# nv-tlabs/DefTet

Measured on AMD Instinct MI355X. Metric: M tet-point tests/s (fwd+bwd) at res=70, 100k queries, higher is better.
Workload: dtype f32

## Files before the change

deftet_amd/csrc/point_in_tet.hip:

```cpp
#pragma clang fp contract(off)

#include <stdlib.h>

#include <algorithm>
#include <type_traits>
#include <vector>

#include "common.hpp"
#include "wave.hpp"

namespace deftet {
namespace pit {

constexpr float kBig = 1048576.0f;
constexpr float kTau = 1.0f / 128.0f;
constexpr float kMargin = 1.0f / 64.0f;
constexpr float kWMin = 9.3132257e-10f;
constexpr int kMiss = 0x7F7F7F7F;
constexpr int kMaxG = 112;
constexpr int kMaxBins = 15 * 1024;
constexpr int kHitOverflow = -2;

constexpr int kHitPad = 64;
__host__ __device__ inline int hit_pad(int B) { return (B + kHitPad - 1) / kHitPad * kHitPad; }
__host__ __device__ inline size_t hit_cnt_off(int B, int T) { return (size_t)B * T * 2; }
__host__ __device__ inline size_t hit_list_off(int B, int T) { return (size_t)B * T * 2 + (size_t)3 * hit_pad(B); }
__host__ __device__ inline size_t hit_spill_off(int B, int T, int Q) { return (hit_list_off(B, T) + (size_t)B * Q + 3) / 4 * 4; }
constexpr int kHitSpilled = 1 << 30;
constexpr int kRecSlots = 2, kSpillSlots = 4;
constexpr int kOvfCap = 128;
__device__ __forceinline__ void note_overflow(int *counters, int nB, int b, int t)
{
    counters[b * 4 + 2] = 1;
    const int k = atomicAdd(&counters[nB * 4 + b * 4 + 2], 1);
    if (k < kOvfCap) counters[nB * 8 + b * kOvfCap + k] = t;
}

__device__ __forceinline__ void put_hit_record(int2 *hits, int4 *spill, size_t idx, const int (&hq)[kRecSlots + kSpillSlots], int n,
                                               int *counters, int nB, int b, int t)
{
    if (n > kRecSlots + kSpillSlots || (n > kRecSlots && !spill)) {
        hits[idx] = make_int2(-1, kHitOverflow);
        note_overflow(counters, nB, b, t);
        return;
    }
    if (n > kRecSlots) spill[idx] = make_int4(hq[2], hq[3], hq[4], hq[5]);
    hits[idx] = make_int2(n > kRecSlots ? (hq[0] | kHitSpilled) : hq[0], hq[1]);
}

#ifdef PIT_PHASE_TIMING
constexpr int kPhaseWaves = 1 << 17;
__device__ unsigned long long g_phase[kPhaseWaves][16];
#define PHASE_DECL                                                                                      \
    long long ph_t_ = clock64();                                                                        \
    const unsigned ph_w_ = (((unsigned)blockIdx.y * gridDim.x + blockIdx.x) * 4u + (threadIdx.x >> 6)) & (kPhaseWaves - 1)
#define PHASE_MARK(i)                                                                  \
    do {                                                                               \
        const long long ph_n_ = clock64();                                             \
        if ((threadIdx.x & 63) == 0) g_phase[ph_w_][i] += (unsigned long long)(ph_n_ - ph_t_); \
        ph_t_ = ph_n_;                                                                 \
    } while (0)
#define PHASE_COUNT(i, v)                                                              \
    do {                                                                               \
        const unsigned long long pc_ = (unsigned long long)(v);                        \
        if ((threadIdx.x & 63) == 0) g_phase[ph_w_][i] += pc_;                         \
    } while (0)
__device__ unsigned long long g_span[kPhaseWaves][2];
#define SPAN_MARK(k)                                                                                                     \
    do {                                                                                                                 \
        if ((threadIdx.x & 63) == 0) g_span[ph_w_][k] = wall_clock64();                                                  \
    } while (0)
__device__ unsigned long long g_reason[8];
#define REASON_COUNT(i, mask)                                                                                        \
    do {                                                                                                             \
        const unsigned long long rm_ = (mask);                                                                       \
        if (rm_ != 0ull && (threadIdx.x & 63) == 0) atomicAdd(&g_reason[i], (unsigned long long)__popcll(rm_));     \
    } while (0)
#else
#define SPAN_MARK(k)
#define REASON_COUNT(i, mask)
#define PHASE_DECL
#define PHASE_MARK(i)
#define PHASE_COUNT(i, v)
#endif

struct Planes {
    float n[4][3];
// ... 160 lines not shown

__device__ __forceinline__ bool query_regular(float x, float y, float z)
{
    return fabsf(x) <= kBig && fabsf(y) <= kBig && fabsf(z) <= kBig;
}

__host__ __device__ inline int table_pitch(int G) { return G + 3; }
__device__ __forceinline__ unsigned table_off(int cz, int cx, int cy, int Gx, int Gp)
{
    return (unsigned)((cz * (Gx + 1) + cx) * Gp + cy);
}

__global__ __launch_bounds__(256) void k_query_bbox(const float *__restrict__ pts, int Q, float *part, int *counters,
                                                    int *result, int nB, long long nQ)
{
    __shared__ float sh[4][6];
    const int b = blockIdx.y;
    {
        const long long nblk = (long long)gridDim.x * gridDim.y, bid = (long long)blockIdx.y * gridDim.x + blockIdx.x;
        const long long i = bid * blockDim.x + threadIdx.x, stride = nblk * blockDim.x;
        if (i < nB * 8) counters[i] = 0;
        for (long long j = i; j < nQ; j += stride) result[j] = kMiss;
    }
    const float *p = pts + (size_t)b * Q * 3;
    float lo[3] = {INFINITY, INFINITY, INFINITY}, hi[3] = {-INFINITY, -INFINITY, -INFINITY};
    constexpr int kBoxKeep = 8;
    const int stride = gridDim.x * blockDim.x;
    for (int q0 = blockIdx.x * blockDim.x + threadIdx.x; q0 < Q; q0 += stride * kBoxKeep) {
        float x[kBoxKeep], y[kBoxKeep], z[kBoxKeep];
#pragma unroll
        for (int k = 0; k < kBoxKeep; ++k) {
            const float *pq = p + (size_t)min(q0 + k * stride, Q - 1) * 3;
            x[k] = pq[0]; y[k] = pq[1]; z[k] = pq[2];
        }
#pragma unroll
        for (int k = 0; k < kBoxKeep; ++k)
            if (query_regular(x[k], y[k], z[k])) {
                lo[0] = fminf(lo[0], x[k]); lo[1] = fminf(lo[1], y[k]); lo[2] = fminf(lo[2], z[k]);
                hi[0] = fmaxf(hi[0], x[k]); hi[1] = fmaxf(hi[1], y[k]); hi[2] = fmaxf(hi[2], z[k]);
            }
    }
#pragma unroll
    for (int off = 32; off > 0; off >>= 1) {
#pragma unroll
        for (int k = 0; k < 3; ++k) {
            lo[k] = fminf(lo[k], __shfl_xor(lo[k], off));
            hi[k] = fmaxf(hi[k], __shfl_xor(hi[k], off));
        }
    }
    const int w = threadIdx.x >> 6;
    if ((threadIdx.x & 63) == 0) {
#pragma unroll
        for (int k = 0; k < 3; ++k) { sh[w][k] = lo[k]; sh[w][3 + k] = hi[k]; }
    }
    __syncthreads();
    if (threadIdx.x < 6) {
        const int k = threadIdx.x;
        float v = sh[0][k];
        for (int i = 1; i < 4; ++i) v = k < 3 ? fminf(v, sh[i][k]) : fmaxf(v, sh[i][k]);
        part[((size_t)b * kBoxBlocks + blockIdx.x) * 6 + k] = v;
    }
}

__device__ __forceinline__ int2 shape_block(int pin)
{
    if (!pin) return make_int2(blockIdx.y, blockIdx.x);
    const int L = blockIdx.y * gridDim.x + blockIdx.x, nB = gridDim.y;
    return make_int2(L % nB, L / nB);
}
static inline int pin_shapes(int Q) { return (size_t)Q * 36 <= ((size_t)4 << 20); }

constexpr int kMaxRowBlocks = 256;
#ifndef PIT_ROWTILE
#define PIT_ROWTILE 2048
#endif
constexpr int kRowTile = PIT_ROWTILE;
#ifndef PIT_LOCAL_THREADS
#define PIT_LOCAL_THREADS 512
#endif
constexpr int kLocalThreads = PIT_LOCAL_THREADS;
constexpr int kLocalWaves = kLocalThreads / 64;
constexpr int kLocalKeep = kRowTile / kLocalThreads;
static_assert(kLocalThreads % 64 == 0 && kLocalKeep * kLocalThreads == kRowTile, "whole waves, whole trips over a chunk");
constexpr int kSub = 4;
constexpr int kParts = 4;
constexpr int kSubPerPart = kSub / kParts;
constexpr int kMaxBin1 = kMaxG * kSub;

template <bool HINT>
__global__ __launch_bounds__(kLocalThreads) void k_slab_local(const float *__restrict__ pts, int Q, const float *__restrict__ bboxPart,
                                                    float *gparam, int G, int Gx, int nblk, int prePitch, int chunkQ,
                                                    float4 *localQ, int *pre, int *counters, int *irregQ,
                                                    const float *__restrict__ boxIn, float *partOut, int *irrCnt, int *result)
{
    __shared__ int hist[kMaxBin1 + 1];
    __shared__ int wtot[kLocalWaves];
    __shared__ int s_irr, s_out;
    __shared__ float s_box[kLocalWaves][6];
    const int b = blockIdx.y, blk = blockIdx.x, R1 = G * kSub, tid = threadIdx.x;
    const int q0 = blk * chunkQ, q1 = min(Q, q0 + chunkQ);
    const bool keep = chunkQ <= kRowTile;
    float3 kp[kLocalKeep];
    if (keep) {
#pragma unroll
        for (int k = 0; k < kLocalKeep; ++k) {
            const float *p = pts + ((size_t)b * Q + max(min(q0 + tid + k * kLocalThreads, q1 - 1), 0)) * 3;
            kp[k] = make_float3(p[0], p[1], p[2]);
        }
    }
    if (HINT) {
        for (int q = q0 + tid; q < q1; q += kLocalThreads) result[(size_t)b * Q + q] = kMiss;
        if (tid == 0) { s_irr = 0; s_out = 0; }
    }
    const Grid g = HINT ? hint_grid(boxIn + (size_t)b * 6, G, Gx) : reduce_grid(bboxPart + (size_t)b * kBoxBlocks * 6, kBoxBlocks, G, Gx);
    float blo[3] = {INFINITY, INFINITY, INFINITY}, bhi[3] = {-INFINITY, -INFINITY, -INFINITY};
    auto box_add = [&](float x, float y, float z) {
        if (HINT && query_regular(x, y, z)) {
            blo[0] = fminf(blo[0], x); blo[1] = fminf(blo[1], y); blo[2] = fminf(blo[2], z);
            bhi[0] = fmaxf(bhi[0], x); bhi[1] = fmaxf(bhi[1], y); bhi[2] = fmaxf(bhi[2], z);
        }
    };
    auto binned = [&](float x, float y, float z) { return HINT ? query_binned(x, y, z, g) : query_regular(x, y, z); };
    auto list_irregular = [&](int q, float x, float y, float z) {
        if (HINT) {
            irregQ[(size_t)b * Q + q0 + atomicAdd(&s_irr, 1)] = q;
            if (query_regular(x, y, z)) atomicAdd(&s_out, 1);
        } else {
            irregQ[(size_t)b * Q + atomicAdd(&counters[b * 4 + 1], 1)] = q;
        }
    };
    if (blk == 0 && tid == 0) {
        float *gp = gparam + b * kGridWords;
#pragma unroll
        for (int k = 0; k < 3; ++k) { gp[k] = g.o[k]; gp[3 + k] = g.inv[k]; gp[6 + k] = g.lo[k]; gp[9 + k] = g.hi[k]; gp[12 + k] = g.pe[k]; gp[15 + k] = g.cs[k]; }
        gp[18] = __int_as_float(wide_cells(g, Q, G, Gx));
        gp[19] = HINT ? 1.0f : 0.f;
    }
    for (int i = tid; i <= R1; i += kLocalThreads) hist[i] = 0;
    __syncthreads();
    const float rcpG = 1.0f / (float)G;
    int kbin[kLocalKeep], krank[kLocalKeep];
    auto bin_of = [&](float x, float y, float z) {
        const int cy = cell_of(y, g.o[1], g.inv[1], G);
        return cell_of(z, g.o[2], g.inv[2], G) * kSub + (int)(((float)(cy * kSub) + 0.5f) * rcpG);
    };
    if (keep) {
#pragma unroll
        for (int k = 0; k < kLocalKeep; ++k) {
            const int q = q0 + tid + k * kLocalThreads;
            kbin[k] = -1;
            if (q < q1) {
                box_add(kp[k].x, kp[k].y, kp[k].z);
                if (binned(kp[k].x, kp[k].y, kp[k].z)) {
                    kbin[k] = bin_of(kp[k].x, kp[k].y, kp[k].z);
                    krank[k] = atomicAdd(&hist[kbin[k]], 1);
                } else {
                    list_irregular(q, kp[k].x, kp[k].y, kp[k].z);
                }
            }
        }
    } else {
        for (int q = q0 + tid; q < q1; q += kLocalThreads) {
            const float *p = pts + ((size_t)b * Q + q) * 3;
            const float x = p[0], y = p[1], z = p[2];
            box_add(x, y, z);
            if (binned(x, y, z)) atomicAdd(&hist[bin_of(x, y, z)], 1);
            else list_irregular(q, x, y, z);
        }
    }
    if (HINT) {
#pragma unroll
        for (int off = 32; off > 0; off >>= 1) {
#pragma unroll
            for (int k = 0; k < 3; ++k) {
                blo[k] = fminf(blo[k], __shfl_xor(blo[k], off));
                bhi[k] = fmaxf(bhi[k], __shfl_xor(bhi[k], off));
            }
        }
        if ((tid & 63) == 0) {
#pragma unroll
            for (int k = 0; k < 3; ++k) { s_box[tid >> 6][k] = blo[k]; s_box[tid >> 6][3 + k] = bhi[k]; }
        }
    }
    __syncthreads();
    if (HINT) {
        if (tid < 6) {
            float v = s_box[0][tid];
            for (int i = 1; i < kLocalWaves; ++i) v = tid < 3 ? fminf(v, s_box[i][tid]) : fmaxf(v, s_box[i][tid]);
            partOut[((size_t)b * kMaxRowBlocks + blk) * 6 + tid] = v;
        }
        if (tid == 0) {
            irrCnt[b * kMaxRowBlocks + blk] = s_irr;
            irrCnt[(gridDim.y + b) * kMaxRowBlocks + blk] = s_out;
        }
    }
    {
        constexpr int kPer = (kMaxBin1 + kLocalThreads - 1) / kLocalThreads;
        const int per = (R1 + kLocalThreads - 1) / kLocalThreads, i0 = tid * per;
        int n[kPer], sum = 0;
#pragma unroll
        for (int j = 0; j < kPer; ++j) {
            n[j] = (j < per && i0 + j < R1) ? hist[i0 + j] : 0;
            sum += n[j];
        }
        const int lane = tid & 63, w = tid >> 6;
        const int incl = wave_incl_sum(sum, lane);
        if (lane == 63) wtot[w] = incl;
        __syncthreads();
        int run = incl - sum;
#pragma unroll
        for (int k = 0; k < kLocalWaves; ++k)
            if (k < w) run += wtot[k];
        int *row = pre + ((size_t)b * nblk + blk) * prePitch;
#pragma unroll
        for (int j = 0; j < kPer; ++j)
            if (j < per && i0 + j < R1) {
                hist[i0 + j] = run;
                row[i0 + j] = run;
                run += n[j];
            }
        if (tid == kLocalThreads - 1) row[R1] = run;
    }
    __syncthreads();
    float4 *dst = localQ + (size_t)b * Q + q0;
    if (keep) {
#pragma unroll
        for (int k = 0; k < kLocalKeep; ++k)
            if (kbin[k] >= 0) dst[hist[kbin[k]] + krank[k]] = make_float4(kp[k].x, kp[k].y, kp[k].z, __int_as_float(q0 + tid + k * kLocalThreads));
    } else {
        for (int q = q0 + tid; q < q1; q += kLocalThreads) {
            const float *p = pts + ((size_t)b * Q + q) * 3;
            const float x = p[0], y = p[1], z = p[2];
            if (binned(x, y, z)) dst[atomicAdd(&hist[bin_of(x, y, z)], 1)] = make_float4(x, y, z, __int_as_float(q));
        }
    }
}

#ifndef PIT_SORT_THREADS
#define PIT_SORT_THREADS 256
#endif
constexpr int kSortThreads = PIT_SORT_THREADS;
constexpr int kSortKeep = 1024 / kSortThreads;
constexpr int kRunsPer = kMaxRowBlocks / kSortThreads;
static_assert(kRunsPer * kSortThreads == kMaxRowBlocks && kSortThreads % 64 == 0, "every chunk run has a thread");
__global__ __launch_bounds__(kSortThreads) void k_slab_sort(const float4 *__restrict__ localQ, int Q, const float *__restrict__ gparam,
                                                            int G, int Gx, const int *__restrict__ pre, int nblk, int prePitch,
                                                            int chunkQ, long long cellStride, int *table, float4 *sortedQ, int pin,
                                                            const float *__restrict__ boxPart, int nPart, int partStride, float *boxOut,
                                                            int hint, const int *__restrict__ irrCnt, int *irregQ, int *counters,
                                                            int *missOut)
{
    if (shape_block(pin).y == 0) {
        const int b0 = shape_block(pin).x, nB = gridDim.y;
        if (boxOut && threadIdx.x < 64) {
            float lo[3], hi[3];
            reduce_box(boxPart + (size_t)b0 * partStride * 6, nPart, lo, hi);
            if (threadIdx.x == 0) {
#pragma unroll
                for (int k = 0; k < 3; ++k) { boxOut[b0 * 6 + k] = lo[k]; boxOut[b0 * 6 + 3 + k] = hi[k]; }
            }
        }
        if (hint && threadIdx.x < 64) {
            int n = 0, nOut = 0;
            for (int c = 0; c < nblk; ++c) {
                const int cnt = irrCnt[b0 * kMaxRowBlocks + c];
                nOut += irrCnt[(nB + b0) * kMaxRowBlocks + c];
                const int *src = irregQ + (size_t)b0 * Q + (size_t)c * chunkQ;
                for (int i = (int)threadIdx.x; i < cnt; i += 64) {
                    const int v = src[i];
                    irregQ[(size_t)b0 * Q + n + i] = v;
                }
                n += cnt;
            }
            if (threadIdx.x == 0) {
                counters[b0 * 4 + 0] = 0; counters[b0 * 4 + 1] = n; counters[b0 * 4 + 2] = 0; counters[b0 * 4 + 3] = 0;
#pragma unroll
                for (int k = 0; k < 4; ++k) counters[nB * 4 + b0 * 4 + k] = 0;
                if (missOut) missOut[b0] = nOut;
            }
        }
        return;
    }
    extern __shared__ __attribute__((aligned(16))) int cnt[];
    __shared__ int wsum[kSortThreads / 64], wsum2[kSortThreads / 64];
    __shared__ int runStart[kMaxRowBlocks + 1], runSrc[kMaxRowBlocks];
    const int2 sb0 = shape_block(pin);
    const int2 sb = make_int2(sb0.x, sb0.y - 1);
    const int b = sb.x, cz = sb.y / kParts, part = sb.y % kParts, tid = threadIdx.x, lane = tid & 63, w = tid >> 6;
    const int GxP = Gx | 1;
    const int cyLo = (part * kSubPerPart * G + kSub - 1) / kSub, cyHi = ((part + 1) * kSubPerPart * G + kSub - 1) / kSub;
    const int nb = (cyHi - cyLo) * GxP;
    const int binLo = cz * kSub + part * kSubPerPart;
    PHASE_DECL;
    SPAN_MARK(0);
    int a[kRunsPer], len[kRunsPer], asum = 0, lsum = 0;
#pragma unroll
    for (int j = 0; j < kRunsPer; ++j) {
        const int r = tid * kRunsPer + j;
        a[j] = 0; len[j] = 0;
        if (r < nblk) {
            const int *row = pre + ((size_t)b * nblk + r) * prePitch + binLo;
            a[j] = row[0];
            len[j] = row[kSubPerPart] - a[j];
        }
        asum += a[j];
        lsum += len[j];
    }
    int s0, n;
    {
        int ia = asum, il = lsum;
#pragma unroll
        for (int off = 1; off < 64; off <<= 1) {
            const int ta = __shfl_up(ia, off), tl = __shfl_up(il, off);
            if (lane >= off) { ia += ta; il += tl; }
        }
        if (lane == 63) { wsum[w] = ia; wsum2[w] = il; }
        __syncthreads();
        int ta = 0, tl = 0, before = 0;
#pragma unroll
        for (int k = 0; k < kSortThreads / 64; ++k) {
            ta += wsum[k];
            tl += wsum2[k];
            if (k < w) before += wsum2[k];
        }
        s0 = ta;
        n = tl;
        int at = before + il - lsum;
#pragma unroll
        for (int j = 0; j < kRunsPer; ++j) {
            const int r = tid * kRunsPer + j;
            if (r < nblk) {
                runStart[r] = at;
                runSrc[r] = r * chunkQ + a[j];
            }
            at += len[j];
        }
        if (tid == 0) runStart[nblk] = n;
    }
    for (int i = tid; i < ((nb + 3) & ~3); i += kSortThreads) cnt[i] = 0;
    __syncthreads();
    const float ox = gparam[b * kGridWords + 0], oy = gparam[b * kGridWords + 1];
    const float ix = gparam[b * kGridWords + 3], iy = gparam[b * kGridWords + 4];
    const int s1 = s0 + n;
    const bool keep = n <= kSortThreads * kSortKeep;
    const float4 *src = localQ + (size_t)b * Q;
    auto source_of = [&](int i) {
        int lo = 0, hi = nblk;
        while (hi - lo > 1) {
            const int mid = (lo + hi) >> 1;
            if (runStart[mid] <= i) lo = mid; else hi = mid;
        }
        return min(runSrc[lo] + (i - runStart[lo]), Q - 1);
    };
    float4 kq[kSortKeep];
    int kbin[kSortKeep], krank[kSortKeep];
    if (keep) {
#pragma unroll
        for (int k = 0; k < kSortKeep; ++k)
            if (k == 0 || k * kSortThreads < n)
                kq[k] = src[source_of(max(min(tid + k * kSortThreads, n - 1), 0))];
    }
    PHASE_MARK(8);
    if (keep) {
#pragma unroll
        for (int k = 0; k < kSortKeep; ++k) {
            if (tid + k * kSortThreads < n) {
                kbin[k] = (cell_of(kq[k].y, oy, iy, G) - cyLo) * GxP + cell_of(kq[k].x, ox, ix, Gx);
                krank[k] = atomicAdd(&cnt[kbin[k]], 1);
            }
        }
    } else {
        for (int i = tid; i < n; i += kSortThreads) {
            const float4 q = src[source_of(i)];
            atomicAdd(&cnt[(cell_of(q.y, oy, iy, G) - cyLo) * GxP + cell_of(q.x, ox, ix, Gx)], 1);
        }
    }
    __syncthreads();
    PHASE_MARK(9);
    {
        const int nb4 = (nb + 3) >> 2;
        const int per = (nb4 + kSortThreads - 1) / kSortThreads, i0 = min(nb4, tid * per), i1 = min(nb4, i0 + per);
        int4 *c4 = reinterpret_cast<int4 *>(cnt);
        int sum = 0;
        for (int i = i0; i < i1; ++i) {
            const int4 v = c4[i];
            sum += (v.x + v.y) + (v.z + v.w);
        }
        const int incl = wave_incl_sum(sum, lane);
        __syncthreads();
        if (lane == 63) wsum[w] = incl;
        __syncthreads();
        int run = s0 + incl - sum;
#pragma unroll
        for (int k = 0; k < kSortThreads / 64; ++k)
            if (k < w) run += wsum[k];
        for (int i = i0; i < i1; ++i) {
            const int4 v = c4[i];
            int4 o;
            o.x = run; o.y = o.x + v.x; o.z = o.y + v.y; o.w = o.z + v.z;
            run = o.w + v.w;
            c4[i] = o;
        }
    }
    __syncthreads();
    PHASE_MARK(10);
    float4 *dst = sortedQ + (size_t)b * Q;
    if (keep) {
#pragma unroll
        for (int k = 0; k < kSortKeep; ++k)
            if (tid + k * kSortThreads < n) dst[cnt[kbin[k]] + krank[k]] = kq[k];
    }
    PHASE_MARK(11);
    {
        const int Gp = table_pitch(G);
        int *tb = table + (size_t)b * cellStride + (size_t)cz * (Gx + 1) * Gp;
        const int cyEnd = part == kParts - 1 ? Gp : cyHi, ny = cyEnd - cyLo;
        const int total = (Gx + 1) * ny, stepx = kSortThreads / ny, stepy = kSortThreads % ny;
        int cx = tid / ny, ry = tid % ny;
        for (int i = tid; i < total; i += kSortThreads) {
            const int cy = cyLo + ry;
            int v;
            if (cy >= G) v = s1;
            else if (cx < Gx) v = cnt[ry * GxP + cx];
            else v = cy + 1 < cyHi ? cnt[(ry + 1) * GxP] : s1;
            tb[cx * Gp + cy] = v;
            cx += stepx;
            ry += stepy;
            if (ry >= ny) { ry -= ny; ++cx; }
        }
    }
    PHASE_MARK(12);
    SPAN_MARK(1);
    if (keep) return;
    __syncthreads();
    for (int i = tid; i < n; i += kSortThreads) {
        const float4 q = src[source_of(i)];
        dst[atomicAdd(&cnt[(cell_of(q.y, oy, iy, G) - cyLo) * GxP + cell_of(q.x, ox, ix, Gx)], 1)] = q;
    }
}

__device__ __forceinline__ void irregular_queries_tail(const Planes &P, int t, int b, int Q, const float *__restrict__ pts,
                                                       const int *__restrict__ counters, const int *__restrict__ irregQ, int *result)
{
    const int n = counters[b * 4 + 1];
    for (int k = 0; k < n; ++k) {
        const int q = irregQ[(size_t)b * Q + k];
        const float *p = pts + ((size_t)b * Q + q) * 3;
        if (accept(P, p[0], p[1], p[2])) atomicMin(&result[(size_t)b * Q + q], t);
    }
}

#ifndef PIT_WAVES
#define PIT_WAVES 5
#endif


struct TetBox {
    float lo[3], hi[3], w;
};
__device__ __forceinline__ bool classify(const float *v, const Planes &P, TetBox &bx)
{
#pragma unroll
    for (int k = 0; k < 3; ++k) {
        bx.lo[k] = fminf(fminf(v[k], v[3 + k]), fminf(v[6 + k], v[9 + k]));
        bx.hi[k] = fmaxf(fmaxf(v[k], v[3 + k]), fmaxf(v[6 + k], v[9 + k]));
    }
    bx.w = fmaxf(fmaxf(bx.hi[0] - bx.lo[0], bx.hi[1] - bx.lo[1]), bx.hi[2] - bx.lo[2]);
    const float big = fmaxf(fmaxf(fmaxf(fabsf(bx.lo[0]), fabsf(bx.hi[0])), fmaxf(fabsf(bx.lo[1]), fabsf(bx.hi[1]))),
                            fmaxf(fabsf(bx.lo[2]), fabsf(bx.hi[2])));
    const float thr = kTau * ((bx.w * bx.w) * bx.w);
    const bool cond = fabsf(P.dv[0]) >= thr && fabsf(P.dv[1]) >= thr && fabsf(P.dv[2]) >= thr && fabsf(P.dv[3]) >= thr;
    return big <= kBig && (P.sv == 0u || P.sv == 15u) && bx.w >= kWMin && cond;
}

struct CellBox {
    int cx0, cx1, cy0, cy1, cz0, cz1;
};

__device__ __forceinline__ float4 ld_f4_hint(const float4 *p, bool nt)
{
    if (!nt) return *p;
    typedef float f4v __attribute__((ext_vector_type(4)));
    const f4v x = __builtin_nontemporal_load(reinterpret_cast<const f4v *>(p));
    return make_float4(x[0], x[1], x[2], x[3]);
}
struct DenseTets {
    typedef const float *__restrict__ Arg;
    typedef const float *Ref;
    typedef const float *__restrict__ RefArg;
    const float *tet;
    __host__ __device__ __forceinline__ DenseTets(const float *p) : tet(p) {}
    __device__ __forceinline__ Ref at(int b, int T, int t) const { return tet + ((size_t)b * T + t) * 12; }
    __device__ __forceinline__ Ref at_flat(long long i, int ) const { return tet + i * 12; }
    template <bool NT = false>
    __device__ __forceinline__ static void get3(Ref r, float4 &a, float4 &bq, float4 &c)
    {
        const float4 *src = reinterpret_cast<const float4 *>(r);
        a = ld_f4_hint(src, NT); bq = ld_f4_hint(src + 1, NT); c = ld_f4_hint(src + 2, NT);
    }
// ... 1872 lines not shown
                                                   int clamp_inplace)
{
    const int b = blockIdx.y;
    const int q = blockIdx.x * blockDim.x + threadIdx.x;
    if (q >= Q) return;
    const size_t i = (size_t)b * Q + q;
    float c = cond[i];
    if (c < 0) {
        c = 0.f;
        if (clamp_inplace) cond[i] = 0.f;
    }
    out[i] = pred[(size_t)b * T + (long long)c];
}

__global__ __launch_bounds__(256) void k_paste_bwd(const float *__restrict__ cond, const float *__restrict__ gout,
                                                   float *gpred, int T, int Q)
{
    const int b = blockIdx.y;
    const int q = blockIdx.x * blockDim.x + threadIdx.x;
    const bool live = q < Q;
    const size_t i = (size_t)b * Q + (live ? q : 0);
    const float c = live ? cond[i] : 0.f;
    const float g = live ? gout[i] : 0.f;
    const bool miss = live && c < 1.0f;
    float gm = miss ? g : 0.f;
#pragma unroll
    for (int off = 32; off > 0; off >>= 1) gm += __shfl_xor(gm, off);
    __shared__ float wsum[4];
    if ((threadIdx.x & 63) == 0) wsum[threadIdx.x >> 6] = gm;
    __syncthreads();
    if (threadIdx.x == 0) {
        const float tot = (wsum[0] + wsum[1]) + (wsum[2] + wsum[3]);
        if (tot != 0.f) unsafeAtomicAdd(&gpred[(size_t)b * T], tot);
    }
    if (live && !miss) unsafeAtomicAdd(&gpred[(size_t)b * T + (long long)c], g);
}

struct Tunables {
    double gdiv = 6.0;
    double qdiv = 2.0;
    double yzfine = 2.0;
    double xfine = 2.0;
    Tunables()
    {
        auto get = [](const char *name, double lo, double hi, double &dst) {
            if (const char *e = getenv(name)) {
                const double v = atof(e);
                if (v >= lo && v <= hi) dst = v;
            }
        };
        get("DEFTET_PIT_GDIV", 0.25, 4096.0, gdiv);
        get("DEFTET_PIT_QDIV", 0.03, 4096.0, qdiv);
        get("DEFTET_PIT_YZFINE", 0.25, 8.0, yzfine);
        get("DEFTET_PIT_XFINE", 0.25, 16.0, xfine);
    }
};
static const Tunables &tunables()
{
    static const Tunables t;
    return t;
}

static int resolve_auto(int algo, int T, int Q)
{
    if (algo != DEFTET_PIT_AUTO) return algo;
    return (double)Q <= 0.6 * (double)T ? DEFTET_PIT_WAVE : DEFTET_PIT_SLAB;
}

static void pick_grid(int T, int Q, int &G, int &Gx)
{
    const Tunables &tn = tunables();
    const double a = T / tn.gdiv, bq = (Q > 0 ? Q : 1) / tn.qdiv;
    const double m = a < bq ? a : bq;
    long long g = llround(tn.yzfine * cbrt(m < 1 ? 1 : m));
    if (g < 1) g = 1;
    if (g > kMaxG) g = kMaxG;
    long long gx = llround(tn.xfine * (double)g);
    if (gx < 1) gx = 1;
    while (gx > 1 && (g / 4 + 2) * (gx | 1) > kMaxBins) --gx;
    G = (int)g;
    Gx = (int)gx;
}

struct Layout {
    int G, Gx, nRowBlk, chunkQ;
    long long cellStride;
    size_t bytes;
    float *bboxPart, *chunkBox;
    int *irrCnt;
    int prePitch;
    int *counters, *table, *pre, *result, *irregT, *irregQ;
    float4 *localQ, *sortedQ;
    float *rec, *gparam;
};

static Layout make_layout(int B, int T, int Q, int algo, void *ws, size_t wsBytes)
{
    Layout L{};
    Arena A(ws, wsBytes);
    L.result = A.take<int>((size_t)B * Q);
    if (algo == DEFTET_PIT_BRUTE) {
        L.rec = A.take<float>((size_t)B * T * 32);
    } else {
        pick_grid(T, Q, L.G, L.Gx);
        const long long n = (long long)L.G * (L.Gx + 1) * table_pitch(L.G);
        L.cellStride = (n + 63) / 64 * 64;
        L.nRowBlk = (Q + kRowTile - 1) / kRowTile;
        if (L.nRowBlk > kMaxRowBlocks) L.nRowBlk = kMaxRowBlocks;
        if (L.nRowBlk < 1) L.nRowBlk = 1;
        L.chunkQ = ((Q + L.nRowBlk - 1) / L.nRowBlk + 255) / 256 * 256;
        L.bboxPart = A.take<float>((size_t)B * kBoxBlocks * 6);
        L.chunkBox = A.take<float>((size_t)B * kMaxRowBlocks * 6);
        L.irrCnt = A.take<int>((size_t)B * kMaxRowBlocks * 2);
        L.counters = A.take<int>((size_t)B * (8 + kOvfCap));
        L.gparam = A.take<float>((size_t)B * kGridWords);
        L.table = A.take<int>((size_t)B * L.cellStride);
        L.prePitch = (L.G * kSub + 1 + 31) / 32 * 32;
        L.pre = A.take<int>((size_t)B * L.nRowBlk * L.prePitch);
        L.localQ = A.take<float4>((size_t)B * Q);
        L.sortedQ = A.take<float4>((size_t)B * Q);
        L.irregT = A.take<int>((size_t)B * T);
        L.irregQ = A.take<int>((size_t)B * Q);
    }
    L.bytes = align_up(A.off, 256);
    return L;
}

}
}

using namespace deftet;
using namespace deftet::pit;

extern "C" size_t deftet_point_in_tet_workspace_bytes(int B, int T, int Q, int algo)
{
    if (B <= 0 || T < 0 || Q < 0) return 0;
    return make_layout(B, T, Q, algo, nullptr, 0).bytes;
}

extern "C" size_t deftet_point_in_tet_hits_ints(int B, int T, int Q)
{
    if (B <= 0 || T < 0 || Q < 0) return 0;
    return hit_spill_off(B, T, Q) + (size_t)B * T * 4;
}

extern "C" int deftet_point_in_tet_resolve_algo(int algo, int T, int Q) { return resolve_auto(algo, T, Q); }

extern "C" int deftet_point_in_tet_grid_dims(int T, int Q, int *G_yz, int *G_x)
{
    DEFTET_CHECK_ARG(T >= 0 && Q >= 0 && G_yz && G_x, "bad argument");
    pick_grid(T, Q, *G_yz, *G_x);
    return DEFTET_OK;
}

static int pit_check(const float *tet, const float *pts, const float *cond, const float *bary, const float *pred, const float *occ,
                     const int32_t *hit_buf, int B, int T, int Q, int algo, const void *workspace)
{
    DEFTET_CHECK_ARG(!hit_buf || (((uintptr_t)hit_buf & 15) == 0 && algo != DEFTET_PIT_BRUTE), "hit_buf must be 16-byte aligned and needs a binned algo");
    DEFTET_CHECK_ARG((pred == nullptr) == (occ == nullptr), "pred and occ must be given together");
    DEFTET_CHECK_ARG(!occ || T > 0, "paste_occ needs at least one tet");
    DEFTET_CHECK_ARG(B >= 0 && T >= 0 && Q >= 0, "negative size (B=%d T=%d Q=%d)", B, T, Q);
    DEFTET_CHECK_ARG(algo == DEFTET_PIT_AUTO || algo == DEFTET_PIT_BRUTE || algo == DEFTET_PIT_EXACT || algo == DEFTET_PIT_SLAB || algo == DEFTET_PIT_WAVE || algo == DEFTET_PIT_PAIR, "unknown algo %d", algo);
    if (T >= (1 << 24)) return set_error(DEFTET_ELIMIT, "n_tet=%d does not fit a float-encoded index (2^24)", T);
    DEFTET_CHECK_ARG(B <= 65535, "n_batch=%d exceeds the grid-y limit 65535", B);
    if (Q >= (1 << 27)) return set_error(DEFTET_ELIMIT, "n_query=%d: 16-byte query records are addressed with 32-bit byte offsets (limit 2^27)", Q);
    if (B == 0 || Q == 0) return DEFTET_OK;
    DEFTET_CHECK_ARG(pts && cond, "null pts/cond pointer");
    DEFTET_CHECK_ARG(T == 0 || tet, "null tet pointer");
    DEFTET_CHECK_ARG(((uintptr_t)tet & 15) == 0, "tet must be 16-byte aligned");
    DEFTET_CHECK_ARG(!bary || ((uintptr_t)bary & 15) == 0, "bary must be 16-byte aligned");
    DEFTET_CHECK_ARG(workspace && ((uintptr_t)workspace & 255) == 0, "workspace null or not 256-byte aligned");
    return DEFTET_OK;
}

static int pit_prepare(const Layout &L, const float *pts, int B, int Q, hipStream_t st, const float *boxIn = nullptr, float *boxOut = nullptr,
                       int32_t *missOut = nullptr)
{
    const dim3 blk(256), lblk(kLocalThreads);
    if (boxIn) {
        DEFTET_LAUNCH(k_slab_local<true>, dim3(L.nRowBlk, B), lblk, st, pts, Q, L.bboxPart, L.gparam, L.G, L.Gx, L.nRowBlk, L.prePitch, L.chunkQ,
                      L.localQ, L.pre, L.counters, L.irregQ, boxIn, L.chunkBox, L.irrCnt, L.result);
    } else {
        DEFTET_LAUNCH(k_query_bbox, dim3(kBoxBlocks, B), blk, st, pts, Q, L.bboxPart, L.counters, L.result, B, (long long)B * Q);
        DEFTET_LAUNCH(k_slab_local<false>, dim3(L.nRowBlk, B), lblk, st, pts, Q, L.bboxPart, L.gparam, L.G, L.Gx, L.nRowBlk, L.prePitch, L.chunkQ,
                      L.localQ, L.pre, L.counters, L.irregQ, (const float *)nullptr, (float *)nullptr, (int *)nullptr, (int *)nullptr);
    }
    const size_t shm = align_up((size_t)((L.G + kParts - 1) / kParts + 1) * (L.Gx | 1) * sizeof(int), 16);
    DEFTET_LAUNCH_SHM(k_slab_sort, dim3(L.G * kParts + 1, B), dim3(kSortThreads), shm, st, L.localQ, Q, L.gparam, L.G, L.Gx, L.pre, L.nRowBlk, L.prePitch,
                      L.chunkQ, L.cellStride, L.table, L.sortedQ, (size_t)Q * 16 <= ((size_t)4 << 20),
                      (const float *)(boxIn ? L.chunkBox : L.bboxPart), boxIn ? L.nRowBlk : kBoxBlocks, boxIn ? kMaxRowBlocks : kBoxBlocks, boxOut,
                      boxIn ? 1 : 0, (const int *)L.irrCnt, L.irregQ, L.counters, (int *)(boxIn ? missOut : nullptr));
    return DEFTET_OK;
}

template <class TS>
static int pit_scan(const Layout &L, typename TS::Arg tet, const float *pts, float *cond, float *bary, const float *pred, float *occ,
                    int32_t *hit_buf, int B, int T, int Q, int algo, hipStream_t st, const int32_t *order = nullptr)
{
    const dim3 blk(256);
    const dim3 gf((Q + 256 * PIT_FIN_QPT - 1) / (256 * PIT_FIN_QPT), B), gt((((T + 255) / 256 + 7) / 8) * 8, B);
    int *ucount = hit_buf ? hit_buf + hit_cnt_off(B, T) : nullptr;
    if (T > 0) {
        if (algo == DEFTET_PIT_EXACT) {
            DEFTET_LAUNCH(k_tet_scan<TS>, gt, blk, st, tet, T, Q, L.gparam, L.G, L.Gx, L.table, L.cellStride, L.sortedQ, L.result,
                          L.counters, L.irregT, (int2 *)hit_buf, pts, L.irregQ, ucount, hit_pad(B), hit_buf ? (int4 *)(hit_buf + hit_spill_off(B, T, Q)) : (int4 *)nullptr);
        } else {
            int4 *spill = hit_buf ? (int4 *)(hit_buf + hit_spill_off(B, T, Q)) : (int4 *)nullptr;
            const int kern = resolve_auto(algo, T, Q);
            const bool slab = kern == DEFTET_PIT_SLAB;
#if PIT_PROBE_SCATTER && PIT_PROBE_PREFILL
            if (spill) DEFTET_HIP(hipMemsetAsync(spill, 0, (size_t)B * Q * 24, st));
#endif
            const dim3 bw(kWvThreads);
            const dim3 gw((((T + kWvThreads - 1) / kWvThreads + 7) / 8) * 8, B);
            const dim3 gp(((((T + 1) / 2 + kWvThreads - 1) / kWvThreads + 7) / 8) * 8, B);
#define PIT_SCAN_ARGS tet, T, Q, L.gparam, L.G, L.Gx, L.table, L.cellStride, L.sortedQ, L.result, L.counters, L.irregT, (int2 *)hit_buf, pts, \
                      L.irregQ, ucount, hit_pad(B), spill, (const int *)order
            typedef TetCfg<TS, true> Ord;
            typedef TetCfg<TS, false> Plain;
            if (slab && order) DEFTET_LAUNCH(k_tet_scan_slab<Ord>, gt, blk, st, PIT_SCAN_ARGS);
            else if (slab) DEFTET_LAUNCH(k_tet_scan_slab<Plain>, gt, blk, st, PIT_SCAN_ARGS);
            else if (kern == DEFTET_PIT_PAIR && order) DEFTET_LAUNCH(k_tet_scan_pair<Ord>, gp, bw, st, PIT_SCAN_ARGS);
            else if (kern == DEFTET_PIT_PAIR) DEFTET_LAUNCH(k_tet_scan_pair<Plain>, gp, bw, st, PIT_SCAN_ARGS);
            else if (order) DEFTET_LAUNCH(k_tet_scan_wave<Ord>, gw, bw, st, PIT_SCAN_ARGS);
            else DEFTET_LAUNCH(k_tet_scan_wave<Plain>, gw, bw, st, PIT_SCAN_ARGS);
#undef PIT_SCAN_ARGS
        }
    } else if (ucount) {
        DEFTET_HIP(hipMemsetAsync(ucount, 0, (size_t)3 * hit_pad(B) * 4, st));
    }
    DEFTET_LAUNCH(k_finalize<TS>, gf, blk, st, tet, pts, T, Q, L.result, cond, bary, pred, occ, (const int2 *)hit_buf, ucount,
                  hit_buf ? hit_buf + hit_list_off(B, T) : nullptr, L.counters, L.irregT, hit_pad(B), pin_shapes(Q), (const float *)L.gparam);
    return DEFTET_OK;
}

template <class TS>
static int pit_forward_checked(typename TS::Arg tet, const float *pts, float *cond, float *bary, const float *pred, float *occ,
                               int32_t *hit_buf, int B, int T, int Q, int algo, void *workspace, size_t workspace_bytes, void *stream_,
                               const int32_t *order, const float *boxIn, float *boxOut, int32_t *missOut)
{
    Layout L = make_layout(B, T, Q, algo, workspace, workspace_bytes);
    DEFTET_CHECK_ARG(L.bytes <= workspace_bytes, "workspace too small: need %zu bytes, got %zu", L.bytes, workspace_bytes);
    hipStream_t st = as_stream(stream_);
    if (algo == DEFTET_PIT_BRUTE) {
        const dim3 blk(256), gq((Q + 255) / 256, B);
        if (T > 0) {
            long long n = (long long)B * T;
            DEFTET_LAUNCH(k_prep_records<TS>, dim3((unsigned)((n + 255) / 256)), blk, st, tet, n, L.rec, T);
        }
        DEFTET_LAUNCH(k_brute, gq, blk, st, L.rec, pts, T, Q, L.result);
        DEFTET_LAUNCH(k_finalize<TS>, dim3((Q + 256 * PIT_FIN_QPT - 1) / (256 * PIT_FIN_QPT), B), blk, st, tet, pts, T, Q, L.result, cond, bary, pred, occ, (const int2 *)nullptr, (int *)nullptr,
                      (int *)nullptr, (const int *)nullptr, L.irregT, 0, pin_shapes(Q), (const float *)nullptr);
        return DEFTET_OK;
    }
    const int rc = pit_prepare(L, pts, B, Q, st, boxIn, boxOut, missOut);
    if (rc != DEFTET_OK) return rc;
    return pit_scan<TS>(L, tet, pts, cond, bary, pred, occ, hit_buf, B, T, Q, algo, st, order);
}
static int pit_forward(const float *tet, const float *pts, float *cond, float *bary, const float *pred, float *occ, int32_t *hit_buf,
                       int B, int T, int Q, int algo, void *workspace, size_t workspace_bytes, void *stream_, const int32_t *order,
                       const float *boxIn = nullptr, float *boxOut = nullptr, int32_t *missOut = nullptr)
{
    int rc = pit_check(tet, pts, cond, bary, pred, occ, hit_buf, B, T, Q, algo, workspace);
    if (rc != DEFTET_OK || B == 0 || Q == 0) return rc;
    return pit_forward_checked<DenseTets>(tet, pts, cond, bary, pred, occ, hit_buf, B, T, Q, algo, workspace, workspace_bytes, stream_, order,
                                          boxIn, boxOut, missOut);
}

extern "C" int deftet_point_in_tet_f32(const float *tet, const float *pts, float *cond, float *bary, const float *pred,
                                       float *occ, int32_t *hit_buf, int B, int T, int Q, int algo, void *workspace,
                                       size_t workspace_bytes, void *stream_)
{
// ... 11 lines not shown
}

static int pit_prepare_entry(const float *pts, int B, int T, int Q, int algo, void *workspace, size_t workspace_bytes, void *stream_,
                             const float *boxIn, float *boxOut, int32_t *missOut);
extern "C" int deftet_point_in_tet_prepare_f32(const float *pts, int B, int T, int Q, int algo, void *workspace,
                                               size_t workspace_bytes, void *stream_)
{
    return pit_prepare_entry(pts, B, T, Q, algo, workspace, workspace_bytes, stream_, nullptr, nullptr, nullptr);
}
extern "C" int deftet_point_in_tet_prepare_ex_f32(const float *pts, int B, int T, int Q, int algo, const float *query_box_in,
                                                  float *query_box_out, int32_t *query_box_misses, void *workspace,
                                                  size_t workspace_bytes, void *stream_)
{
    DEFTET_CHECK_ARG(!query_box_in || query_box_in != query_box_out, "query_box_in and query_box_out must not alias");
    return pit_prepare_entry(pts, B, T, Q, algo, workspace, workspace_bytes, stream_, query_box_in, query_box_out, query_box_misses);
}
static int pit_prepare_entry(const float *pts, int B, int T, int Q, int algo, void *workspace, size_t workspace_bytes, void *stream_,
                             const float *boxIn, float *boxOut, int32_t *missOut)
{
    DEFTET_CHECK_ARG(B >= 0 && T >= 0 && Q >= 0 && B <= 65535, "bad size (B=%d T=%d Q=%d)", B, T, Q);
    DEFTET_CHECK_ARG(algo == DEFTET_PIT_AUTO || algo == DEFTET_PIT_EXACT || algo == DEFTET_PIT_SLAB || algo == DEFTET_PIT_WAVE || algo == DEFTET_PIT_PAIR, "prepare needs a binned algo (got %d)", algo);
    if (Q >= (1 << 27)) return set_error(DEFTET_ELIMIT, "n_query=%d exceeds 2^27", Q);
    if (B == 0 || Q == 0) return DEFTET_OK;
    DEFTET_CHECK_ARG(pts, "null pts pointer");
    DEFTET_CHECK_ARG(workspace && ((uintptr_t)workspace & 255) == 0, "workspace null or not 256-byte aligned");
    Layout L = make_layout(B, T, Q, algo, workspace, workspace_bytes);
    DEFTET_CHECK_ARG(L.bytes <= workspace_bytes, "workspace too small: need %zu bytes, got %zu", L.bytes, workspace_bytes);
    return pit_prepare(L, pts, B, Q, as_stream(stream_), boxIn, boxOut, missOut);
}

static int pit_scan_entry(const float *tet, const float *pts, float *cond, float *bary, const float *pred, float *occ, int32_t *hit_buf,
                          int B, int T, int Q, int algo, void *workspace, size_t workspace_bytes, void *stream_, const int32_t *order)
{
    DEFTET_CHECK_ARG(algo != DEFTET_PIT_BRUTE, "scan needs a binned algo");
    int rc = pit_check(tet, pts, cond, bary, pred, occ, hit_buf, B, T, Q, algo, workspace);
    if (rc != DEFTET_OK || B == 0 || Q == 0) return rc;
    Layout L = make_layout(B, T, Q, algo, workspace, workspace_bytes);
    DEFTET_CHECK_ARG(L.bytes <= workspace_bytes, "workspace too small: need %zu bytes, got %zu", L.bytes, workspace_bytes);
    return pit_scan<DenseTets>(L, tet, pts, cond, bary, pred, occ, hit_buf, B, T, Q, algo, as_stream(stream_), order);
}

extern "C" int deftet_point_in_tet_scan_f32(const float *tet, const float *pts, float *cond, float *bary, const float *pred,
                                            float *occ, int32_t *hit_buf, int B, int T, int Q, int algo, void *workspace,
                                            size_t workspace_bytes, void *stream_)
{
    return pit_scan_entry(tet, pts, cond, bary, pred, occ, hit_buf, B, T, Q, algo, workspace, workspace_bytes, stream_, nullptr);
}

extern "C" int deftet_point_in_tet_scan_ex_f32(const float *tet, const float *pts, float *cond, float *bary, const float *pred,
                                                    float *occ, int32_t *hit_buf, int B, int T, int Q, int algo,
                                                    const int32_t *tet_order, void *workspace, size_t workspace_bytes, void *stream_)
{
    return pit_scan_entry(tet, pts, cond, bary, pred, occ, hit_buf, B, T, Q, algo, workspace, workspace_bytes, stream_, tet_order);
}

extern "C" int deftet_point_in_tet_read_stats(const void *workspace, size_t workspace_bytes, int B, int T, int Q, int algo,
                                              int32_t *out_host, void *stream_)
{
    DEFTET_CHECK_ARG(workspace && out_host && B > 0 && algo != DEFTET_PIT_BRUTE, "bad argument");
    Layout L = make_layout(B, T, Q, algo, const_cast<void *>(workspace), workspace_bytes);
    DEFTET_CHECK_ARG(L.bytes <= workspace_bytes, "workspace too small");
    hipStream_t st = as_stream(stream_);
    std::vector<int32_t> tmp((size_t)B * 8);
    DEFTET_HIP(hipMemcpyAsync(tmp.data(), L.counters, (size_t)B * 32, hipMemcpyDeviceToHost, st));
    DEFTET_HIP(hipStreamSynchronize(st));
    for (int b = 0; b < B; ++b)
        for (int k = 0; k < 4; ++k) {
            out_host[b * 8 + k] = tmp[(size_t)b * 4 + k];
            out_host[b * 8 + 4 + k] = tmp[(size_t)B * 4 + (size_t)b * 4 + k];
        }
    return DEFTET_OK;
}

extern "C" int deftet_debug_point_in_tet_layout(int B, int T, int Q, int algo, long long *out8)
{
    DEFTET_CHECK_ARG(out8 && B > 0 && T >= 0 && Q >= 0 && algo != DEFTET_PIT_BRUTE, "bad argument");
    const Layout L = make_layout(B, T, Q, algo, nullptr, 0);
    auto off = [](const void *p) { return (long long)reinterpret_cast<uintptr_t>(p); };
    out8[0] = L.G; out8[1] = L.Gx; out8[2] = L.cellStride;
    out8[3] = off(L.gparam); out8[4] = off(L.table); out8[5] = off(L.sortedQ); out8[6] = off(L.counters); out8[7] = off(L.irregQ);
    return DEFTET_OK;
}

#ifdef PIT_PHASE_TIMING
extern "C" int deftet_debug_occupancy(int *out8)
{
    int n = 0;
    DEFTET_HIP(hipOccupancyMaxActiveBlocksPerMultiprocessor(&n, (const void *)deftet::pit::k_tet_scan_wave<deftet::pit::TetCfg<deftet::pit::DenseTets, false>>, 256, 0)); out8[0] = n;
    DEFTET_HIP(hipOccupancyMaxActiveBlocksPerMultiprocessor(&n, (const void *)deftet::pit::k_tet_scan_pair<deftet::pit::TetCfg<deftet::pit::DenseTets, false>>, 256, 0)); out8[1] = n;
    DEFTET_HIP(hipOccupancyMaxActiveBlocksPerMultiprocessor(&n, (const void *)deftet::pit::k_tet_scan_slab<deftet::pit::TetCfg<deftet::pit::DenseTets, false>>, 256, 0)); out8[2] = n;
    hipFuncAttributes a;
    DEFTET_HIP(hipFuncGetAttributes(&a, (const void *)deftet::pit::k_tet_scan_wave<deftet::pit::TetCfg<deftet::pit::DenseTets, false>>));
    out8[3] = (int)a.sharedSizeBytes; out8[4] = a.numRegs; out8[5] = (int)a.maxDynamicSharedSizeBytes;
    hipDeviceProp_t pr;
    DEFTET_HIP(hipGetDeviceProperties(&pr, 0));
    out8[6] = (int)pr.sharedMemPerMultiprocessor; out8[7] = (int)pr.sharedMemPerBlock;
    return DEFTET_OK;
}
extern "C" int deftet_debug_span_read(unsigned long long *out, int n_waves)
{
    DEFTET_CHECK_ARG(out && n_waves > 0 && n_waves <= deftet::pit::kPhaseWaves, "bad argument");
    DEFTET_HIP(hipMemcpyFromSymbol(out, HIP_SYMBOL(deftet::pit::g_span), (size_t)n_waves * 16));
    return DEFTET_OK;
}
extern "C" int deftet_debug_reason_read(unsigned long long *out8, int reset)
{
    DEFTET_HIP(hipMemcpyFromSymbol(out8, HIP_SYMBOL(deftet::pit::g_reason), 64));
    if (reset) {
        unsigned long long z[8] = {0};
        DEFTET_HIP(hipMemcpyToSymbol(HIP_SYMBOL(deftet::pit::g_reason), z, 64));
    }
    return DEFTET_OK;
}
extern "C" int deftet_debug_phase_read(unsigned long long *out16, int reset)
{
    std::vector<unsigned long long> h((size_t)kPhaseWaves * 16);
    DEFTET_HIP(hipMemcpyFromSymbol(h.data(), HIP_SYMBOL(deftet::pit::g_phase), h.size() * sizeof(unsigned long long)));
    for (int i = 0; i < 16; ++i) out16[i] = 0;
    for (size_t w = 0; w < (size_t)kPhaseWaves; ++w)
        for (int i = 0; i < 16; ++i) out16[i] += h[w * 16 + i];
    if (reset) {
        std::fill(h.begin(), h.end(), 0ull);
        DEFTET_HIP(hipMemcpyToSymbol(HIP_SYMBOL(deftet::pit::g_phase), h.data(), h.size() * sizeof(unsigned long long)));
    }
    return DEFTET_OK;
}
#endif

constexpr long long kDenseQueriesPerTet = 2;
extern "C" size_t deftet_point_in_tet_bwd_workspace_bytes(int B, int T, int Q)
{
    if (B <= 0 || T < 0 || Q < 0) return 0;
    const size_t lists = align_up((size_t)B * T * 4, 256) + align_up((size_t)B * Q * 4, 256) + align_up((size_t)B * 4, 256);
    const size_t miss = align_up((size_t)B * kMissStride * 4, 256);
    return lists > miss ? lists : miss;
}

static bool tets_null(const float *tet) { return tet == nullptr; }
static bool tets_null(const IndexedTets &s) { return s.pos == nullptr || s.idx == nullptr; }
static bool tets_misaligned(const float *tet) { return ((uintptr_t)tet & 15) != 0; }
static bool tets_misaligned(const IndexedTets &s) { return ((uintptr_t)s.idx & 15) != 0 || ((uintptr_t)s.pos & 3) != 0; }

template <class TS>
static int pit_bwd(typename TS::Arg tet, const float *pts, const float *cond, const float *grad_w, float *grad_tet, float *grad_pts,
                   const float *grad_occ, float *grad_pred, const int32_t *hit_buf, int B, int T, int Q, int accumulate, void *workspace,
                   size_t workspace_bytes, void *stream_)
{
    DEFTET_CHECK_ARG(B >= 0 && T >= 0 && Q >= 0, "negative size");
    DEFTET_CHECK_ARG(B <= 65535, "n_batch=%d exceeds 65535", B);
    DEFTET_CHECK_ARG((grad_occ == nullptr) == (grad_pred == nullptr), "grad_occ and grad_pred must be given together");
    hipStream_t st = as_stream(stream_);
    if (B == 0) return DEFTET_OK;
    if (grad_pts && Q > 0) DEFTET_HIP(hipMemsetAsync(grad_pts, 0, (size_t)B * Q * 12, st));
    if (T == 0) return DEFTET_OK;
    DEFTET_CHECK_ARG(grad_tet && ((uintptr_t)grad_tet & 15) == 0, "grad_tet null or not 16-byte aligned");
    if (Q == 0) {
        if (!accumulate) {
            DEFTET_HIP(hipMemsetAsync(grad_tet, 0, (size_t)B * T * 48, st));
            if (grad_pred) DEFTET_HIP(hipMemsetAsync(grad_pred, 0, (size_t)B * T * 4, st));
        }
        return DEFTET_OK;
    }
    DEFTET_CHECK_ARG(!tets_null(tet) && pts && cond && grad_w, "null pointer");
    DEFTET_CHECK_ARG(!tets_misaligned(tet) && ((uintptr_t)grad_w & 15) == 0, "tet/grad_w must be 16-byte aligned");
    const bool dense = (long long)Q > kDenseQueriesPerTet * (long long)T && workspace && ((uintptr_t)workspace & 255) == 0 &&
                       workspace_bytes >= deftet_point_in_tet_bwd_workspace_bytes(B, T, Q);
// ... 218 lines not shown
```

Baseline: 1.082 billion.

## Choose query-sort part count from occupancy and parallelize irregular-list compaction

Measured after the change: 1.089 billion, median of 6. About the same (+0.7%).

```diff
diff --git a/deftet_amd/csrc/point_in_tet.hip b/deftet_amd/csrc/point_in_tet.hip
--- a/deftet_amd/csrc/point_in_tet.hip
+++ b/deftet_amd/csrc/point_in_tet.hip
@@ -3,6 +3,7 @@
 #include <stdlib.h>
 
 #include <algorithm>
+#include <mutex>
 #include <type_traits>
 #include <vector>
 
@@ -329,14 +330,12 @@
 constexpr int kLocalWaves = kLocalThreads / 64;
 constexpr int kLocalKeep = kRowTile / kLocalThreads;
 static_assert(kLocalThreads % 64 == 0 && kLocalKeep * kLocalThreads == kRowTile, "whole waves, whole trips over a chunk");
-constexpr int kSub = 4;
-constexpr int kParts = 4;
-constexpr int kSubPerPart = kSub / kParts;
-constexpr int kMaxBin1 = kMaxG * kSub;
+constexpr int kMaxParts = 4;
+constexpr int kMaxBin1 = kMaxG * kMaxParts;
 
 template <bool HINT>
 __global__ __launch_bounds__(kLocalThreads) void k_slab_local(const float *__restrict__ pts, int Q, const float *__restrict__ bboxPart,
-                                                    float *gparam, int G, int Gx, int nblk, int prePitch, int chunkQ,
+                                                    float *gparam, int G, int Gx, int nblk, int prePitch, int nParts, int chunkQ,
                                                     float4 *localQ, int *pre, int *counters, int *irregQ,
                                                     const float *__restrict__ boxIn, float *partOut, int *irrCnt, int *result)
 {
@@ -344,7 +343,7 @@
     __shared__ int wtot[kLocalWaves];
     __shared__ int s_irr, s_out;
     __shared__ float s_box[kLocalWaves][6];
-    const int b = blockIdx.y, blk = blockIdx.x, R1 = G * kSub, tid = threadIdx.x;
+    const int b = blockIdx.y, blk = blockIdx.x, R1 = G * nParts, tid = threadIdx.x;
     const int q0 = blk * chunkQ, q1 = min(Q, q0 + chunkQ);
     const bool keep = chunkQ <= kRowTile;
     float3 kp[kLocalKeep];
@@ -389,7 +388,7 @@
     int kbin[kLocalKeep], krank[kLocalKeep];
     auto bin_of = [&](float x, float y, float z) {
         const int cy = cell_of(y, g.o[1], g.inv[1], G);
-        return cell_of(z, g.o[2], g.inv[2], G) * kSub + (int)(((float)(cy * kSub) + 0.5f) * rcpG);
+        return cell_of(z, g.o[2], g.inv[2], G) * nParts + (int)(((float)(cy * nParts) + 0.5f) * rcpG);
     };
     if (keep) {
 #pragma unroll
@@ -491,41 +490,63 @@
 constexpr int kRunsPer = kMaxRowBlocks / kSortThreads;
 static_assert(kRunsPer * kSortThreads == kMaxRowBlocks && kSortThreads % 64 == 0, "every chunk run has a thread");
 __global__ __launch_bounds__(kSortThreads) void k_slab_sort(const float4 *__restrict__ localQ, int Q, const float *__restrict__ gparam,
-                                                            int G, int Gx, const int *__restrict__ pre, int nblk, int prePitch,
+                                                            int G, int Gx, const int *__restrict__ pre, int nblk, int prePitch, int nParts,
                                                             int chunkQ, long long cellStride, int *table, float4 *sortedQ, int pin,
                                                             const float *__restrict__ boxPart, int nPart, int partStride, float *boxOut,
                                                             int hint, const int *__restrict__ irrCnt, int *irregQ, int *counters,
                                                             int *missOut)
 {
     if (shape_block(pin).y == 0) {
-        const int b0 = shape_block(pin).x, nB = gridDim.y;
-        if (boxOut && threadIdx.x < 64) {
+        if (threadIdx.x >= 64) return;
+        const int b0 = shape_block(pin).x, nB = gridDim.y, lane = threadIdx.x;
+        PHASE_DECL;
+        SPAN_MARK(0);
+        constexpr int kCntPasses = kMaxRowBlocks / 64;
+        int cnt[kCntPasses], out[kCntPasses];
+#pragma unroll
+        for (int p = 0; p < kCntPasses; ++p) {
+            const int c = p * 64 + lane;
+            const bool has = hint && c < nblk;
+            cnt[p] = has ? irrCnt[b0 * kMaxRowBlocks + c] : 0;
+            out[p] = has ? irrCnt[(nB + b0) * kMaxRowBlocks + c] : 0;
+        }
+        if (boxOut) {
             float lo[3], hi[3];
             reduce_box(boxPart + (size_t)b0 * partStride * 6, nPart, lo, hi);
-            if (threadIdx.x == 0) {
+            if (lane == 0) {
 #pragma unroll
                 for (int k = 0; k < 3; ++k) { boxOut[b0 * 6 + k] = lo[k]; boxOut[b0 * 6 + 3 + k] = hi[k]; }
             }
         }
-        if (hint && threadIdx.x < 64) {
+        if (hint) {
             int n = 0, nOut = 0;
-            for (int c = 0; c < nblk; ++c) {
-                const int cnt = irrCnt[b0 * kMaxRowBlocks + c];
-                nOut += irrCnt[(nB + b0) * kMaxRowBlocks + c];
-                const int *src = irregQ + (size_t)b0 * Q + (size_t)c * chunkQ;
-                for (int i = (int)threadIdx.x; i < cnt; i += 64) {
-                    const int v = src[i];
-                    irregQ[(size_t)b0 * Q + n + i] = v;
+#pragma unroll
+            for (int p = 0; p < kCntPasses; ++p) {
+                if (p * 64 < nblk) {
+                    const int start = n + wave_incl_sum(cnt[p], lane) - cnt[p];
+                    lanemask_t m = __ballot(cnt[p] > 0);
+                    while (m) {
+                        const int l = __ffsll((long long)m) - 1;
+                        m &= m - 1;
+                        const int len = lane_bcast(cnt[p], l), at = lane_bcast(start, l);
+                        const int *src = irregQ + (size_t)b0 * Q + (size_t)(p * 64 + l) * chunkQ;
+                        for (int i = lane; i < len; i += 64) {
+                            const int v = src[i];
+                            irregQ[(size_t)b0 * Q + at + i] = v;
+                        }
+                    }
+                    n += wave_sum(cnt[p]);
+                    nOut += wave_sum(out[p]);
                 }
-                n += cnt;
-            }
-            if (threadIdx.x == 0) {
+            }
+            if (lane == 0) {
                 counters[b0 * 4 + 0] = 0; counters[b0 * 4 + 1] = n; counters[b0 * 4 + 2] = 0; counters[b0 * 4 + 3] = 0;
 #pragma unroll
                 for (int k = 0; k < 4; ++k) counters[nB * 4 + b0 * 4 + k] = 0;
                 if (missOut) missOut[b0] = nOut;
             }
         }
+        SPAN_MARK(1);
         return;
     }
     extern __shared__ __attribute__((aligned(16))) int cnt[];
@@ -533,11 +554,12 @@
     __shared__ int runStart[kMaxRowBlocks + 1], runSrc[kMaxRowBlocks];
     const int2 sb0 = shape_block(pin);
     const int2 sb = make_int2(sb0.x, sb0.y - 1);
-    const int b = sb.x, cz = sb.y / kParts, part = sb.y % kParts, tid = threadIdx.x, lane = tid & 63, w = tid >> 6;
+    const int b = sb.x, cz = sb.y / nParts, part = sb.y % nParts, tid = threadIdx.x, lane = tid & 63, w = tid >> 6;
+    const float gpw = gparam[b * kGridWords + (lane & 7)];
     const int GxP = Gx | 1;
-    const int cyLo = (part * kSubPerPart * G + kSub - 1) / kSub, cyHi = ((part + 1) * kSubPerPart * G + kSub - 1) / kSub;
+    const int cyLo = (part * G + nParts - 1) / nParts, cyHi = ((part + 1) * G + nParts - 1) / nParts;
     const int nb = (cyHi - cyLo) * GxP;
-    const int binLo = cz * kSub + part * kSubPerPart;
+    const int binLo = cz * nParts + part;
     PHASE_DECL;
     SPAN_MARK(0);
     int a[kRunsPer], len[kRunsPer], asum = 0, lsum = 0;
@@ -548,11 +570,12 @@
         if (r < nblk) {
             const int *row = pre + ((size_t)b * nblk + r) * prePitch + binLo;
             a[j] = row[0];
-            len[j] = row[kSubPerPart] - a[j];
+            len[j] = row[1] - a[j];
         }
         asum += a[j];
         lsum += len[j];
     }
+    const float ox = lane_bcast(gpw, 0), oy = lane_bcast(gpw, 1), ix = lane_bcast(gpw, 3), iy = lane_bcast(gpw, 4);
     int s0, n;
     {
         int ia = asum, il = lsum;
@@ -586,8 +609,6 @@
     }
     for (int i = tid; i < ((nb + 3) & ~3); i += kSortThreads) cnt[i] = 0;
     __syncthreads();
-    const float ox = gparam[b * kGridWords + 0], oy = gparam[b * kGridWords + 1];
-    const float ix = gparam[b * kGridWords + 3], iy = gparam[b * kGridWords + 4];
     const int s1 = s0 + n;
     const bool keep = n <= kSortThreads * kSortKeep;
     const float4 *src = localQ + (size_t)b * Q;
@@ -661,7 +682,7 @@
     {
         const int Gp = table_pitch(G);
         int *tb = table + (size_t)b * cellStride + (size_t)cz * (Gx + 1) * Gp;
-        const int cyEnd = part == kParts - 1 ? Gp : cyHi, ny = cyEnd - cyLo;
+        const int cyEnd = part == nParts - 1 ? Gp : cyHi, ny = cyEnd - cyLo;
         const int total = (Gx + 1) * ny, stepx = kSortThreads / ny, stepy = kSortThreads % ny;
         int cx = tid / ny, ry = tid % ny;
         for (int i = tid; i < total; i += kSortThreads) {
@@ -2700,6 +2721,51 @@
     Gx = (int)gx;
 }
 
+static int pre_pitch(int G, int P) { return (G * P + 1 + 31) / 32 * 32; }
+static size_t sort_counters(int G, int Gx, int P) { return (size_t)((G + P - 1) / P + 1) * (Gx | 1); }
+static size_t sort_shm(int G, int Gx, int P) { return align_up(sort_counters(G, Gx, P) * sizeof(int), 16); }
+
+constexpr int kXcds = 8;
+struct SortPlan {
+    int P, perShape, slots, rounds;
+};
+static int g_forceParts = 0;
+static int sort_plan(int B, int G, int Gx, bool pin, SortPlan &out)
+{
+    struct Entry {
+        int dev, B, G, Gx, pin, force;
+        SortPlan plan;
+    };
+    static std::mutex mu;
+    static std::vector<Entry> cache;
+    int dev = 0;
+    DEFTET_HIP(hipGetDevice(&dev));
+    const int force = g_forceParts;
+    std::lock_guard<std::mutex> lock(mu);
+    for (const Entry &e : cache)
+        if (e.dev == dev && e.B == B && e.G == G && e.Gx == Gx && e.pin == (int)pin && e.force == force) {
+            out = e.plan;
+            return DEFTET_OK;
+        }
+    int cus = 0;
+    DEFTET_HIP(hipDeviceGetAttribute(&cus, hipDeviceAttributeMultiprocessorCount, dev));
+    SortPlan best{0, 0, 0, 0};
+    for (int P = kMaxParts; P >= 1; --P) {
+        if ((force && P != force) || sort_counters(G, Gx, P) > (size_t)kMaxBins) continue;
+        int perCu = 0;
+        DEFTET_HIP(hipOccupancyMaxActiveBlocksPerMultiprocessor(&perCu, (const void *)k_slab_sort, kSortThreads, sort_shm(G, Gx, P)));
+        const long long wgs = (long long)B * (G * P + 1);
+        const long long slots = (long long)(perCu > 0 ? perCu : 1) * (pin ? (cus >= kXcds ? cus / kXcds : 1) : cus);
+        const long long mine = pin ? (wgs + kXcds - 1) / kXcds : wgs;
+        const long long rounds = (mine + slots - 1) / slots;
+        if (best.P == 0 || rounds < best.rounds) best = SortPlan{P, G * P + 1, (int)slots, (int)rounds};
+    }
+    if (best.P == 0) return set_error(DEFTET_EINVAL, "no part count fits the query sort's counters (G=%d Gx=%d forced=%d)", G, Gx, force);
+    cache.push_back(Entry{dev, B, G, Gx, (int)pin, force, best});
+    out = best;
+    return DEFTET_OK;
+}
+
 struct Layout {
     int G, Gx, nRowBlk, chunkQ;
     long long cellStride;
@@ -2733,7 +2799,7 @@
         L.counters = A.take<int>((size_t)B * (8 + kOvfCap));
         L.gparam = A.take<float>((size_t)B * kGridWords);
         L.table = A.take<int>((size_t)B * L.cellStride);
-        L.prePitch = (L.G * kSub + 1 + 31) / 32 * 32;
+        L.prePitch = pre_pitch(L.G, kMaxParts);
         L.pre = A.take<int>((size_t)B * L.nRowBlk * L.prePitch);
         L.localQ = A.take<float4>((size_t)B * Q);
         L.sortedQ = A.take<float4>((size_t)B * Q);
@@ -2795,17 +2861,21 @@
                        int32_t *missOut = nullptr)
 {
     const dim3 blk(256), lblk(kLocalThreads);
+    const bool pin = (size_t)Q * 16 <= ((size_t)4 << 20);
+    SortPlan plan;
+    const int rcPlan = sort_plan(B, L.G, L.Gx, pin, plan);
+    if (rcPlan != DEFTET_OK) return rcPlan;
+    const int P = plan.P, prePitch = pre_pitch(L.G, P);
     if (boxIn) {
-        DEFTET_LAUNCH(k_slab_local<true>, dim3(L.nRowBlk, B), lblk, st, pts, Q, L.bboxPart, L.gparam, L.G, L.Gx, L.nRowBlk, L.prePitch, L.chunkQ,
+        DEFTET_LAUNCH(k_slab_local<true>, dim3(L.nRowBlk, B), lblk, st, pts, Q, L.bboxPart, L.gparam, L.G, L.Gx, L.nRowBlk, prePitch, P, L.chunkQ,
                       L.localQ, L.pre, L.counters, L.irregQ, boxIn, L.chunkBox, L.irrCnt, L.result);
     } else {
         DEFTET_LAUNCH(k_query_bbox, dim3(kBoxBlocks, B), blk, st, pts, Q, L.bboxPart, L.counters, L.result, B, (long long)B * Q);
-        DEFTET_LAUNCH(k_slab_local<false>, dim3(L.nRowBlk, B), lblk, st, pts, Q, L.bboxPart, L.gparam, L.G, L.Gx, L.nRowBlk, L.prePitch, L.chunkQ,
+        DEFTET_LAUNCH(k_slab_local<false>, dim3(L.nRowBlk, B), lblk, st, pts, Q, L.bboxPart, L.gparam, L.G, L.Gx, L.nRowBlk, prePitch, P, L.chunkQ,
                       L.localQ, L.pre, L.counters, L.irregQ, (const float *)nullptr, (float *)nullptr, (int *)nullptr, (int *)nullptr);
     }
-    const size_t shm = align_up((size_t)((L.G + kParts - 1) / kParts + 1) * (L.Gx | 1) * sizeof(int), 16);
-    DEFTET_LAUNCH_SHM(k_slab_sort, dim3(L.G * kParts + 1, B), dim3(kSortThreads), shm, st, L.localQ, Q, L.gparam, L.G, L.Gx, L.pre, L.nRowBlk, L.prePitch,
-                      L.chunkQ, L.cellStride, L.table, L.sortedQ, (size_t)Q * 16 <= ((size_t)4 << 20),
+    DEFTET_LAUNCH_SHM(k_slab_sort, dim3(L.G * P + 1, B), dim3(kSortThreads), sort_shm(L.G, L.Gx, P), st, L.localQ, Q, L.gparam, L.G, L.Gx, L.pre, L.nRowBlk,
+                      prePitch, P, L.chunkQ, L.cellStride, L.table, L.sortedQ, pin ? 1 : 0,
                       (const float *)(boxIn ? L.chunkBox : L.bboxPart), boxIn ? L.nRowBlk : kBoxBlocks, boxIn ? kMaxRowBlocks : kBoxBlocks, boxOut,
                       boxIn ? 1 : 0, (const int *)L.irrCnt, L.irregQ, L.counters, (int *)(boxIn ? missOut : nullptr));
     return DEFTET_OK;
@@ -2983,6 +3053,24 @@
     return DEFTET_OK;
 }
 
+extern "C" int deftet_debug_point_in_tet_force_parts(int parts)
+{
+    DEFTET_CHECK_ARG(parts >= 0 && parts <= kMaxParts, "parts must be 0 (automatic) .. %d", kMaxParts);
+    g_forceParts = parts;
+    return DEFTET_OK;
+}
+extern "C" int deftet_debug_point_in_tet_sort_plan(int B, int T, int Q, int algo, int *out4)
+{
+    DEFTET_CHECK_ARG(out4 && B > 0 && T >= 0 && Q >= 0 && algo != DEFTET_PIT_BRUTE, "bad argument");
+    int G, Gx;
+    pick_grid(T, Q, G, Gx);
+    SortPlan plan;
+    const int rc = sort_plan(B, G, Gx, (size_t)Q * 16 <= ((size_t)4 << 20), plan);
+    if (rc != DEFTET_OK) return rc;
+    out4[0] = plan.P; out4[1] = plan.perShape; out4[2] = plan.slots; out4[3] = plan.rounds;
+    return DEFTET_OK;
+}
+
 #ifdef PIT_PHASE_TIMING
 extern "C" int deftet_debug_occupancy(int *out8)
 {
```
